# BaeHann/feature_level_style_transfer_for_TSC

Hardware: AMD Instinct MI355X
Metric: train-step samples/sec (univariate TS, len=512, batch=256) at 1/2/4/8 MI355X (higher is better)
Workload: dtype bf16x3

## Files before the change

### feature_level_style_transfer_for_tsc_amd/_lib.py

```python
from __future__ import annotations

import ctypes
import os
from ctypes import POINTER, Structure, c_char_p, c_float, c_int, c_int32, c_int64, c_void_p
from typing import Optional

import torch

ABI_VERSION = 21
_LIB_NAME = "libfst_hip.so"
_HERE = os.path.dirname(os.path.abspath(__file__))
LIB_PATH = os.environ.get("FST_HIP_LIB", os.path.join(_HERE, _LIB_NAME))


class FstLibraryError(RuntimeError):
    pass


class WSrc(Structure):
    _fields_ = [("w", c_void_p), ("off0", c_int64), ("sm", c_int64), ("sc", c_int64), ("st", c_int64)]


_P = c_void_p
_I32P = c_void_p
_SIGNATURES = {
    "fst_version": (c_int, []),
    "fst_last_error": (c_char_p, []),
    "fst_pack_weights": (c_int, [_I32P, _I32P, c_int, POINTER(WSrc), POINTER(WSrc), c_int, c_int, c_int, c_int, _P, c_void_p]),
    "fst_pack_weights_bf16x3": (c_int, [_I32P, _I32P, c_int, POINTER(WSrc), POINTER(WSrc), c_int, c_int, c_int, c_int, _P, c_void_p]),
    "fst_unpack_weights": (c_int, [_I32P, _I32P, c_int, _P, c_int, _P, c_int64, c_int64, c_int64, c_int64,
                                   _P, c_int64, c_int64, c_int64, c_int64, c_int, c_void_p]),
    "fst_mask_taps": (c_int, [_P, _I32P, _I32P, c_int, c_int, c_int, c_void_p]),
    "fst_conv_gemm": (c_int, [_P, c_int64, _P, c_int64, _P, _I32P, _I32P, c_int, _P, _P, c_int64, _P, c_int64,
                              _P, c_int64, c_int, c_int, c_int, c_int, c_int, c_int, c_int, c_int, c_void_p]),
    "fst_conv_wgrad": (c_int, [_P, c_int64, _P, c_int64, _P, c_int64, _P, c_int64, c_int, _P, _I32P, _I32P, c_int,
                               c_int, c_int, c_int, c_int, c_int, c_int64, c_void_p]),
    "fst_conv_last_route": (c_int, [POINTER(c_int32)]),
    "fst_row_sum": (c_int, [_P, c_int64, c_int, c_int, c_int, _P, c_void_p]),
    "fst_bn_stats": (c_int, [_P, c_int, c_int, c_int, _P, c_int64, c_void_p]),
    "fst_bn_finalize": (c_int, [_P, c_int, _P, _P, _P, _P, c_int, c_int, c_float, c_float, _P, c_void_p]),
    "fst_bn_apply": (c_int, [_P, _P, _P, _P, _P, c_int, c_int, c_int, c_int, c_int64, c_void_p]),
    "fst_bn_bwd_reduce": (c_int, [_P, _P, _P, _P, c_int, c_int, c_int, c_int, _P, c_int64, c_void_p]),
    "fst_bn_bwd_apply": (c_int, [_P, _P, _P, _P, _P, c_int, _P, _P, _P, c_int, c_int, c_int, c_int, c_int, c_int, c_int64, c_void_p]),
    "fst_bn_bwd_reduce_join": (c_int, [_P, _P, _P, _P, _P, c_int, c_int, c_int, _P, _P, c_int64, c_void_p]),
    "fst_bn_bwd_apply_join": (c_int, [_P, _P, _P, _P, _P, _P, _P, c_int, _P, _P, _P, _P, _P, _P, c_int, c_int, c_int, c_int, c_int,
                                      c_int64, c_void_p]),
    "fst_gate_fwd": (c_int, [_P, _P, c_int, c_int, c_int, c_int64, c_void_p]),
    "fst_gate_bwd": (c_int, [_P, _P, _P, c_int, c_int, c_int, c_int64, c_void_p]),
    "fst_coupling_sum_slots": (c_int64, [c_int, c_int, c_int]),
    "fst_coupling_fwd": (c_int, [_P, _P, _P, c_int, c_int, c_int, c_int64, _P, c_void_p]),
    "fst_coupling_bwd": (c_int, [_P, _P, _P, _P, _P, _P, _P, _P, c_int, c_int, c_int, c_int64, c_void_p]),
    "fst_coupling_inv_fwd": (c_int, [_P, _P, _P, c_int, c_int, c_int, c_int64, c_void_p]),
    "fst_coupling_inv_bwd": (c_int, [_P, _P, _P, _P, _P, c_int, c_int, c_int, c_int64, c_void_p]),
    "fst_rmsprop_multi": (c_int, [_P, _P, _P, _P, _P, c_int, c_float, c_float, c_void_p]),
    "fst_adam_multi": (c_int, [_P, _P, _P, _P, _P, c_int, _P, c_float, c_float, c_float, c_float, c_void_p]),
    "fst_rmsprop_multi_dev": (c_int, [_P, _P, _P, _P, _P, c_int, c_float, c_float, c_void_p]),
    "fst_adam_multi_dev": (c_int, [_P, _P, _P, _P, _P, c_int, _P, _P, c_float, c_float, c_float, c_void_p]),
# ... 129 lines not shown
```

### feature_level_style_transfer_for_tsc_amd/csrc/conv_engine.hip

```cpp
#include "fst_device.h"
#include <algorithm>
#include <type_traits>

struct ConvGemmParams {
  const float* x[2];
  long long x_bs[2];
  const float* a;
  const int32_t* plan;
  const float* bias;
  float* y;
  long long y_bs;
  const float* res;
  long long res_bs;
  float* y2;
  long long y2_bs;
  int msplit, m2_start;
  int B, L, M;
  int tiles_per_seq, ksplit, flags, mg_per_wg, ldw;
  int stage_vec;
  int epi_vec;
  int epi_lds_off;
};

template <int MB, int NB, int MODE>
// ... 439 lines not shown
    asm volatile("s_waitcnt vmcnt(0)" ::: "memory");
#endif
    FST_T(td);
    FST_ACC(3, tc, td);
    if (qn < ct.q_end) commit(buf ^ 1);
    FST_T(te);
    FST_ACC(4, td, te);
    __syncthreads();
    FST_T(tf);
    FST_ACC(5, te, tf);
    q = qn;
    buf ^= 1;
  }
  FST_T(tg);

  conv_epilogue<MB, NB>(p, acc, g, ct.b, ct.t0, ct.wave_n0, ct.half, ct.l31, p.bias != nullptr && blockIdx.z == 0, lds);
  FST_T(th);
  FST_ACC(6, tg, th);
  FST_ACC(7, ts0, th);
  FST_FLUSH(fst_stamps);
}

template <int MB, int NB>
__global__ __launch_bounds__(256, 2) void conv_gemm_bf3_kernel(ConvGemmParams p, const int32_t* __restrict__ plan) {
  extern __shared__ __attribute__((aligned(16))) float lds[];
  constexpr int TILE_N = 128 * NB;
  constexpr int NBLK = TILE_N / 32 + 1;
  constexpr int GS = NBLK * 1024 + 128;
  constexpr int A_BYTES = MB * 2048;
  constexpr int SLOT = A_BYTES + 2 * GS;
  constexpr int NA = A_BYTES / 1024;
  constexpr int NI = NA + 2 * NBLK;
  constexpr int NPW = (NI + 3) / 4;
  char* const ldsb = reinterpret_cast<char*>(lds);
  const PlanView pv = plan_view(plan);
  const ConvTile ct = conv_tile<TILE_N, NB>(p, pv);
  const int tid = ct.tid, lane = ct.lane, half = ct.half, l31 = ct.l31, b = ct.b, t0 = ct.t0, q_begin = ct.q_begin, q_end = ct.q_end,
            wave_n0 = ct.wave_n0;
  const int g = blockIdx.y;
  const int L = p.L;
  const int32_t* ent = pv.mg + 4 * (g * pv.n_chunks);
  const int wave_s = __builtin_amdgcn_readfirstlane(tid >> 6);
  const char* const zero16 = reinterpret_cast<const char*>(p.a) + (long long)pv.n_stages * A_BYTES;

  auto issue = [&](int q, int slot) {
    const int32_t* c = pv.chunk + 4 * q;
    const int32_t* e = ent + 4 * q;
    const int c_count = c[2];
    const char* asrc = reinterpret_cast<const char*>(p.a) + (long long)e[3] * A_BYTES;
    const float* xb = p.x[c[0]] + (long long)b * p.x_bs[c[0]] + (long long)c[1] * L;
    const int tbase = t0 - pv.pad_left + e[0] * pv.dil;
    const int t4 = tbase & ~3;
    const bool spill = (tbase & 3) != 0;
    char* const sl = ldsb + slot * SLOT;
#pragma unroll
    for (int i = 0; i < NPW; ++i) {
      const int idx = wave_s + 4 * i;
      if (idx >= NI) break;
      if (idx < NA) {
        lds_dma16(asrc + idx * 1024 + lane * 16, sl + idx * 1024);
      } else {
        const int bi = idx - NA;
        const int gq = bi >= NBLK ? 1 : 0, m = bi - gq * NBLK;
        const int row = 8 * gq + (lane >> 3);
        const int t = t4 + 32 * m + 4 * (lane & 7);
        bool ok = row < c_count && t >= 0 && t < L;
        if (m == NBLK - 1) ok = ok && spill && (lane & 7) == 0;
        const char* src = ok ? reinterpret_cast<const char*>(xb + ((long long)row * L + t)) : zero16;
        lds_dma16(src, sl + A_BYTES + gq * GS + m * 1024);
      }
    }
  };
  auto wait_stage = [&](int newer) {
    constexpr int R = NI % 4;
    const bool full = R == 0 || wave_s < R;
    if (newer == 0) wait_vmcnt<0>();
    else if (newer == 1) { if (full) wait_vmcnt<NPW>(); else wait_vmcnt<NPW - 1>(); }
    else { if (full) wait_vmcnt<2 * NPW>(); else wait_vmcnt<2 * NPW - 2>(); }
  };

  f32x16 acc[MB][NB];
  zero_acc(acc);

  FST_SUMS(8);
  FST_T(ts0);
  int q0 = next_live(ent, q_begin, q_end);
  int q1 = q0 < q_end ? next_live(ent, q0 + 1, q_end) : q_end;
  if (q0 < q_end) issue(q0, 0);
  if (q1 < q_end) issue(q1, 1);
  int slot = 0;
  FST_T(ts1);
  FST_ACC(0, ts0, ts1);
  while (q0 < q_end) {
    FST_T(ta);
    const int q2 = q1 < q_end ? next_live(ent, q1 + 1, q_end) : q_end;
    wait_stage(q1 < q_end ? 1 : 0);
    FST_T(tb);
    FST_ACC(1, ta, tb);
    __builtin_amdgcn_s_barrier();
    FST_T(tc);
    FST_ACC(2, tb, tc);
    if (q2 < q_end) issue(q2, slot >= 1 ? slot - 1 : 2);
    FST_T(td);
    FST_ACC(3, tc, td);
    const int sub = (t0 - pv.pad_left + ent[4 * q0] * pv.dil) & 3;
    const char* base = ldsb + slot * SLOT;
    bf16x8 bh[NB], bl[NB];
#pragma unroll
    for (int nb = 0; nb < NB; ++nb) {
      const int colx = wave_n0 + nb * 32 + l31 + sub;
      const char* bp = base + A_BYTES + half * GS + (colx >> 5) * 1024 + (colx & 31) * 4;
      float v[8];
#pragma unroll
      for (int j = 0; j < 8; ++j) v[j] = *reinterpret_cast<const float*>(bp + j * 128);
      split_bf16x8(v, bh[nb], bl[nb]);
    }
#ifdef FST_STAMPS
    asm volatile("" ::"v"(bh[0]), "v"(bl[0]), "v"(bh[NB - 1]), "v"(bl[NB - 1]));
#endif
    FST_T(te);
    FST_ACC(4, td, te);
#pragma unroll
    for (int mb = 0; mb < MB; ++mb) {
      bf16x8 ah, al;
      lds_read_a_frag(base, mb, lane, ah, al);
#pragma unroll
      for (int nb = 0; nb < NB; ++nb) mfma_bf3(acc[mb][nb], ah, al, bh[nb], bl[nb]);
    }
    FST_T(tf);
    FST_ACC(5, te, tf);
    q0 = q1;
    q1 = q2;
    slot = slot == 2 ? 0 : slot + 1;
  }
  FST_T(tg);
  __syncthreads();
  conv_epilogue<MB, NB>(p, acc, g, b, t0, wave_n0, half, l31, p.bias != nullptr && blockIdx.z == 0, lds);
  FST_T(th);
  FST_ACC(6, tg, th);
  FST_ACC(7, ts0, th);
  FST_FLUSH(fst_stamps);
}

template <int MB, int NB>
__global__ __launch_bounds__(256, 2) void conv_win_bf3_kernel(ConvGemmParams p, const int32_t* __restrict__ plan) {
  extern __shared__ __attribute__((aligned(16))) float lds[];
  constexpr int TILE_N = 128 * NB;
  char* const ldsb = reinterpret_cast<char*>(lds);
  const PlanView pv = plan_view(plan);
  const ConvTile ct = conv_tile<TILE_N, NB>(p, pv);
  const int g_begin = blockIdx.y * p.mg_per_wg;
  const int g_end = min(pv.n_mgroups, g_begin + p.mg_per_wg);
  const int slot_bytes = p.ldw * 64;

  const bool resident = p.stage_vec != 0;
  int jlo_all = 0, width_all = 0;
  if (resident) {
    conv_window_union(pv, ct.q_begin, ct.q_end, g_begin, g_end, TILE_N, jlo_all, width_all);
    for (int q = ct.q_begin; q < ct.q_end; ++q)
      stage_window_bf16(p, pv, ct, q, jlo_all, width_all, ldsb + (q - ct.q_begin) * slot_bytes);
    __syncthreads();
  }

// ... 376 lines not shown
                     fst_aligned16(res);
  ConvRoute r;
  if (int rc = conv_gemm_route(pv, ps, nb_cfg, L, ksplit, flags, in16, out16, res != nullptr, &r)) return rc;

  ConvGemmParams p;
  p.x[0] = x0; p.x[1] = x1; p.x_bs[0] = x0_bs; p.x_bs[1] = x1_bs;
  p.a = a_packed; p.plan = plan_dev; p.bias = bias;
  p.y = y; p.y_bs = y_bs; p.res = res; p.res_bs = res_bs; p.y2 = y2; p.y2_bs = y2_bs; p.msplit = msplit;
  p.m2_start = m2_start;
  p.B = B; p.L = L; p.M = M;
  p.tiles_per_seq = (L + 128 * nb_cfg - 1) / (128 * nb_cfg);
  p.ksplit = ksplit; p.flags = flags;
  p.mg_per_wg = r.mg_per_wg; p.ldw = r.ldw; p.stage_vec = r.stage_vec; p.epi_vec = r.epi_vec; p.epi_lds_off = r.epi_lds_off;
  if (r.lds_bytes > 48 * 1024)
    if (int rc = fst_allow_full_lds((const void*)r.fn, "fst_conv_gemm")) return rc;
  const bool rows = r.family == FST_ROUTE_WIN_ROWS;
  set_route(r.family, rows ? 0 : pv.MB, rows ? 0 : nb_cfg, r.vec, 0, 0, r.epi, ksplit);
  dim3 grid((unsigned)(B * p.tiles_per_seq), (unsigned)((pv.n_mgroups + r.mg_per_wg - 1) / r.mg_per_wg), (unsigned)ksplit);
  hipLaunchKernelGGL(r.fn, grid, dim3(256), r.lds_bytes, (hipStream_t)stream, p, plan_dev);
  FST_LAUNCH_CHECK();
  return 0;
}

struct WgradParams {
  const float* x[2];
  long long x_bs[2];
  const float* dy;
  long long dy_bs;
  const float* dy2;
  long long dy2_bs;
  int msplit;
  float* da;
  const int32_t* plan;
  int B, L, M, ksplit, tiles_per_seq, ldw, region_floats, n_regions;
  long long x0_mul_off;
  long long slab_floats;
};

#define WG_ITEMS 4

__device__ __forceinline__ int wg_wave_u(int tid) { return __builtin_amdgcn_readfirstlane(tid >> 6); }

template <int MBW, int TW, bool VEC, bool BF3>
struct WgDyStage {
  static constexpr int DYS = TW + 1;
  static constexpr int DYB = 2 * TW + 16;
// ... 682 lines not shown
```

### feature_level_style_transfer_for_tsc_amd/csrc/fst_device.h

```cpp
#pragma once
#include "fst_common.h"

typedef __bf16 bf16x8 __attribute__((ext_vector_type(8)));
typedef __bf16 bf16x2 __attribute__((ext_vector_type(2)));
typedef float f32x2 __attribute__((ext_vector_type(2)));
typedef unsigned u32x4 __attribute__((ext_vector_type(4)));
typedef float f32x16 __attribute__((ext_vector_type(16)));

__device__ __forceinline__ void split_bf16_pair(float a, float b, unsigned& hi, unsigned& lo) {
  const f32x2 v = {a, b};
  hi = __builtin_bit_cast(unsigned, __builtin_convertvector(v, bf16x2));
  const f32x2 r = {a - __uint_as_float(hi << 16), b - __uint_as_float(hi & 0xffff0000u)};
  lo = __builtin_bit_cast(unsigned, __builtin_convertvector(r, bf16x2));
}

__device__ __forceinline__ void split_bf16x8(const float (&v)[8], bf16x8& hi, bf16x8& lo) {
  u32x4 h, l;
#pragma unroll
  for (int j = 0; j < 4; ++j) {
    unsigned hh, ll;
    split_bf16_pair(v[2 * j], v[2 * j + 1], hh, ll);
    h[j] = hh; l[j] = ll;
  }
  hi = __builtin_bit_cast(bf16x8, h);
// ... 31 lines not shown
  asm volatile("s_waitcnt vmcnt(%0)" ::"n"(N) : "memory");
}

__device__ __forceinline__ void lds_dma16(const void* gsrc, void* lds_dst) {
  __builtin_amdgcn_global_load_lds((const __attribute__((address_space(1))) void*)gsrc, (__attribute__((address_space(3))) void*)lds_dst,
                                   16, 0, 0);
}

#ifdef FST_STAMPS
__device__ __forceinline__ unsigned long long fst_now() {
  unsigned long long t;
  asm volatile("s_memtime %0\n\ts_waitcnt lgkmcnt(0)" : "=s"(t)::"memory");
  return t;
}
template <int N>
int fst_read_stamps(unsigned long long (&counters)[N], unsigned long long* out_host, int reset) {
  if (out_host) hipMemcpyFromSymbol(out_host, HIP_SYMBOL(counters), sizeof(counters));
  if (reset) { unsigned long long z[N] = {0}; hipMemcpyToSymbol(HIP_SYMBOL(counters), z, sizeof(z)); }
  return 0;
}
#define FST_T(var) const unsigned long long var = fst_now()
#define FST_ACC(slot, a, b) fst_sum_[slot] += (b) - (a)
#define FST_SUMS(N) unsigned long long fst_sum_[N] = {0}
#define FST_FLUSH(counters) \
  if (lane == 0) for (int i_ = 0; i_ < (int)(sizeof(fst_sum_) / sizeof(fst_sum_[0])); ++i_) atomicAdd(&counters[i_], fst_sum_[i_])
#else
#define FST_T(var)
#define FST_ACC(slot, a, b)
#define FST_SUMS(N)
#define FST_FLUSH(counters)
#endif
```

### feature_level_style_transfer_for_tsc_amd/ops.py

```python
from __future__ import annotations

import ctypes
import math
import os
from typing import Callable, Dict, List, NamedTuple, Optional, Sequence, Tuple

import torch

from . import _lib
from . import dist as _dist
from ._lib import WSrc, check, ptr, stream_ptr
from .plan import Plan, Segment, build_plan, pick_mb

EPI_RELU, EPI_ACC2, EPI_ATOMIC, EPI_ACC1 = 1, 2, 4, 8
GEMM_BF16X3 = 16
WGRAD_SLABS = 32
MATH = os.environ.get("FST_MATH", "bf16x3")
LDS_BUDGET = 96 * 1024
LDS_MULTI_CHUNK = 44 * 1024
PIPE_C = 16

_PARTIAL_BACKWARD = False


# ... 206 lines not shown
        flags |= GEMM_BF16X3
    msplit = M if msplit is None else msplit
    m2_start = msplit if m2_start is None else m2_start
    x0_bs, _ = _ncl(x0, "x0")
    x1_bs = _ncl(x1, "x1")[0] if x1 is not None else 0
    y_bs = _ncl(y, "y")[0] if y is not None else 0
    res_bs = _ncl(res, "res")[0] if res is not None else 0
    y2_bs = _ncl(y2, "y2")[0] if y2 is not None else 0
    t0 = KERNEL_TIMER.begin() if KERNEL_TIMER is not None else None
    check(lib.fst_conv_gemm(ptr(x0), x0_bs, ptr(x1), x1_bs, ptr(a), ptr(plan.dev(x0.device)), plan.host_ptr(),
                            plan.length, ptr(bias), ptr(y), y_bs, ptr(res), res_bs, ptr(y2), y2_bs, msplit, m2_start, B, L,
                            M, nb, ksplit, flags, stream_ptr()), "fst_conv_gemm")
    if t0 is not None:
        key = route_kernel_name(last_route())
        if KERNEL_TIMER.detail:
            key += f" M={M} rec={plan.total_records} dil={plan.dil}"
        rows_in = x0.size(1) + (x1.size(1) if x1 is not None else 0) + (res.size(1) if res is not None else 0)
        rows_out = (msplit if y is not None else 0) + ((M - m2_start) if y2 is not None else 0)
        if y2 is not None and flags & EPI_ACC2:
            rows_in += M - m2_start
        if flags & EPI_ACC1 and y is not None:
            rows_in += msplit
        KERNEL_TIMER.end(key, t0, 2.0 * B * L * _plan_macs_per_step(plan, M), 4.0 * B * L * (rows_in + rows_out))


def conv_wgrad(plan: Plan, x0: Tensor, x1: Optional[Tensor], dy: Tensor, dy2: Optional[Tensor], msplit: int, B: int,
               L: int, M: int, ksplit: int, x0_mul_off: int = 0) -> Tensor:
    lib = _lib.load()
    n_slabs = max(1, min(ksplit, B * ((L + 31) // 32)))
    da = torch.empty(n_slabs, plan.packed_floats, device=x0.device, dtype=torch.float32)
    x0_bs, _ = _ncl(x0, "x0")
    x1_bs = _ncl(x1, "x1")[0] if x1 is not None else 0
    dy_bs, _ = _ncl(dy, "dy")
    dy2_bs = _ncl(dy2, "dy2")[0] if dy2 is not None else 0
    t0 = KERNEL_TIMER.begin() if KERNEL_TIMER is not None else None
    bf3 = MATH == "bf16x3"
    check(lib.fst_conv_wgrad(ptr(x0), x0_bs, ptr(x1), x1_bs, ptr(dy), dy_bs, ptr(dy2), dy2_bs, msplit, ptr(da),
                             ptr(plan.dev(x0.device)), plan.host_ptr(), plan.length, B, L, M, ksplit,
                             (GEMM_BF16X3 if bf3 else 0) | WGRAD_SLABS, x0_mul_off, stream_ptr()),
          "fst_conv_wgrad")
    if t0 is not None:
        key = route_kernel_name(last_route())
        if KERNEL_TIMER.detail:
            key += f" M={M} rec={plan.total_records} ksplit={ksplit}"
        rows_in = x0.size(1) + (x1.size(1) if x1 is not None else 0) + M
        KERNEL_TIMER.end(key, t0, 2.0 * B * L * _plan_macs_per_step(plan, M), 4.0 * B * L * rows_in + 8.0 * plan.packed_floats)
# ... 1220 lines not shown
                                        _ptr_table(da_out), rs_b, rs_d, ptr(do), h2, do.numel(), ptr(d_u0), d_u0_bs, nl, B, L, n, h,
                                        numel, stream_ptr()), "fst_wn_stack_bwd_proj")
    else:
        check(lib.fst_wn_stack_bwd(_ptr_table(ts_list), _ptr_table(imgs_b), _ptr_table(imgs_d), _ptr_table(dgs), _ptr_table(da_out),
                                   rs_b, rs_d, ptr(d_out), ptr(d_u0), d_u0_bs, nl, B, L, n, h, numel, stream_ptr()),
              "fst_wn_stack_bwd")
    if t0 is not None:
        sr = n if do is None else h2
        flops = 2.0 * B * L * (n * ((n + sr) * nl - n) + nl * 2 * n * (3 * n + h))
        rows = nl * (2 * n + sr + 2 * 2 * n + 2 * h) + n * sum(t is not None for t in da_out)
        KERNEL_TIMER.end("wn_stack_bwd_kernel", t0, flops, 4.0 * B * L * rows)


def _wn_layer(S: WNSpecs, ts: Sequence[Tensor], i: int):
    n, nl = S.n, S.n_layers
    rows = slice(2 * n * i, 2 * n * (i + 1))
    return ts[6 + i], ts[2][rows], ts[6 + nl + i], ts[3][rows], ts[6 + 2 * nl + i], ts[6 + 3 * nl + i]


def wn_infer_enabled() -> bool:
    return os.environ.get("FST_WN_INFER", "1") != "0"


def _wn_forward(specs: WNSpecs, u0: Tensor, flat: Tensor, save: bool = True):
    S, nl, n, h = specs, specs.n_layers, specs.n, specs.h
    flat = flat.contiguous()
    W = S.unflatten(flat)
    B, _, L = u0.shape
    dev = u0.device
    infer = not save and wn_infer_enabled()
    y0 = torch.empty(B, n, L, device=dev, dtype=torch.float32) if infer else empty_with_slack(B, n, L, dev)
    a = S.start.forward(u0, None, W[0], None, W[1], y=y0)
    fused = wn_fused_ok(n, h, L, a, u0, kernel=S.kernel)
    if fused:
        out = torch.empty(B, n, L, device=dev, dtype=torch.float32)
        imgs = wn_pack_layers([_wn_layer(S, W, i) for i in range(nl)], n, h)
        if infer:
            other = torch.empty_like(a) if nl > 1 else None
            a_list, ts_list = [a if i % 2 == 0 else other for i in range(nl)], None
        else:
            a_list = [a] + [empty_with_slack(B, n, L, dev) for _ in range(nl - 1)]
            ts_list = [torch.empty(B, 2 * n, L, device=dev, dtype=torch.float32) for _ in range(nl)]
        if wn_stack_fwd_ok(n, h, L, nl, B):
            _wn_stack_forward(not infer, a_list, u0, imgs, ts_list or (), out, n, h)
        else:
            for i in range(nl):
                last = i == nl - 1
                _wn_layer_forward(not infer, a_list[i], u0, imgs[i], ts_list[i] if ts_list else None, None,
                                  None if last else a_list[i + 1], out, i == 0, last, n, h, 2 ** i)
        if infer:
            return S.end.forward(out, None, W[4], None, W[5]), True, ()
        acts_list = ts_list
    else:
        lib = _lib.load()
        out = torch.zeros(B, n, L, device=dev, dtype=torch.float32)
        bias_g = torch.stack(W[6 + nl: 6 + 2 * nl]) + W[3].view(nl, 2 * n)
        a_list, ts_list, acts_list = [a], [], []
        for i in range(nl):
            in_w, cond_w, _, _, rs_w, rs_b = _wn_layer(S, W, i)
            g = S.ins[i].forward(a, u0, in_w, cond_w, bias_g[i])
            acts = torch.empty(B, n, L, device=dev, dtype=torch.float32)
            check(lib.fst_gate_fwd(ptr(g), ptr(acts), B, n, L, _gate_numel(acts, g), stream_ptr()), "fst_gate_fwd")
            ts_list.append(g)
            acts_list.append(acts)
            if i < nl - 1:
                a_next = torch.empty_like(a)
                S.rs[i].forward(acts, None, rs_w, None, rs_b, y=a_next, res=a, y2=out, msplit=n, flags=EPI_ACC2)
                a = a_next
                a_list.append(a)
            else:
                S.rs[i].forward(acts, None, rs_w, None, rs_b, y=None, y2=out, msplit=0, flags=EPI_ACC2)
    o = S.end.forward(out, None, W[4], None, W[5])
    return o, fused, (u0, out, *a_list, *ts_list, *acts_list, flat)


def _wn_backward(S: WNSpecs, fused: bool, sv, do: Tensor, d_u0: Tensor, need_w: bool, pool: Optional["WNGradPool"] = None):
    nl, h, n = S.n_layers, S.h, S.n
    u0, out, flat = sv[0], sv[1], sv[2 + 3 * nl]
    a_list, ts_list, acts_list = sv[2: 2 + nl], sv[2 + nl: 2 + 2 * nl], sv[2 + 2 * nl: 2 + 3 * nl]
    W = S.unflatten(flat)
    B, _, L = u0.shape
    deferring = need_w and pool is not None and fused and any(
        wn_wgrad_ok(0, B, L, n, h, 2 ** i, a_list[i]) or wn_wgrad_ok(1, B, L, n, h, 2 ** i) for i in range(nl))
    d_flat = (torch.zeros_like(flat) if deferring else torch.empty_like(flat)) if need_w else None
    G = S.unflatten(d_flat) if need_w else None
    do = do.contiguous()

    stack = fused and all(wn_dgrad_ok(n, h, 2 ** i) for i in range(nl)) and wn_stack_bwd_ok(n, h, L, nl)
    proj = stack and wn_skip_proj_ok(h, need_w)
    d_out = None if proj and not need_w else S.end.grad_x0(do, W[4])
    da_sums = None
    if need_w:
        S.end.grad_w(out, None, do, out0=G[4])
        row_sum(do, out=G[5])
        d_out_sum = row_sum(d_out, out=G[6 + 4 * nl - 1])
        o0 = S.offsets[6 + 3 * nl]
        d_rs_b = d_flat[o0: o0 + (nl - 1) * 2 * n].view(nl - 1, 2 * n)
        d_rs_b[:, n:] = d_out_sum
        da_sums = [G[1]] + [d_rs_b[i, :n] for i in range(nl - 1)]
    part_b = part_d = None
    if not fused:
        d_a = _wn_backward_unfused(S, W, G, a_list, ts_list, acts_list, u0, d_out, d_u0, da_sums)
    elif stack:
        d_a, part_b, part_d = _wn_backward_stack(S, W, G, a_list, ts_list, u0, d_out, d_u0, pool, do if proj else None)
    else:
        d_a, part_b, part_d = _wn_backward_layers(S, W, G, a_list, ts_list, u0, d_out, d_u0, da_sums, pool)
    S.start.grad_x0(d_a, W[0], out=d_u0, flags=EPI_ACC1)
    if need_w:
        S.start.grad_w(u0, None, d_a, out0=G[0])
        o0 = S.offsets[6 + nl]
        if part_b is not None:
            torch.sum(part_b[:, : 2 * n, :], dim=2, out=d_flat[o0: o0 + nl * 2 * n].view(nl, 2 * n))
        if part_d is not None:
            if nl > 1:
                torch.sum(part_d[1:, :n, :], dim=2, out=d_rs_b[:, :n])
            torch.sum(part_d[0, :n, :], dim=1, out=G[1])
        G[3].copy_(d_flat[o0: o0 + nl * 2 * n])
    return d_flat


def _wn_wgrad_rs(S: WNSpecs, i: int, d_a: Optional[Tensor], d_out: Tensor, ts: Tensor, G, pool) -> None:
    n, B, L, last, g_rs_w = S.n, d_out.size(0), d_out.size(2), i == S.n_layers - 1, _wn_layer(S, G, i)[4]
    if wn_wgrad_ok(1, B, L, n, S.h, 2 ** i):
        if pool is not None:
            pool.add((1, i), (d_a, d_out, ts))
        else:
            wn_wgrad_rs(d_a, d_out, ts, g_rs_w, last, n)
    elif last:
        S.rs[i].grad_w(ts[:, :n], None, d_out, x0_mul_off=n * L, out0=g_rs_w)
    else:
# ... 183 lines not shown

    @staticmethod
    def backward(ctx, dxn, d_o_ext, g_ls, g_sq):
        lib = _lib.load()
        keep, o = ctx.saved_tensors[0], ctx.saved_tensors[1]
        sv = ctx.saved_tensors[2:]
        S: WNSpecs = ctx.specs
        B, C, L = keep.shape
        if ctx.inverse:
            if dxn is None:
                dx, d_o = torch.zeros_like(keep), torch.zeros_like(o)
            else:
                dx, d_o = torch.empty_like(keep), torch.empty_like(o)
                dxn = dxn.contiguous()
                check(lib.fst_coupling_inv_bwd(ptr(keep), ptr(o), ptr(dxn), ptr(dx), ptr(d_o), B, S.h, L,
                                               _same_numel(keep, o, dxn, dx, d_o), stream_ptr()), "fst_coupling_inv_bwd")
        else:
            dx, d_o = _coupling_backward(keep, o, dxn, g_ls, g_sq)
        if d_o_ext is not None:
            d_o = d_o + d_o_ext
        need_w = ctx.needs_input_grad[2] and _want_weight_grad()
        d_flat = _wn_backward(S, ctx.fused, sv, d_o, dx[:, : S.h], need_w, ctx.pool)
        return None, (dx if ctx.needs_input_grad[1] else None), d_flat, None, None


class CouplingInvFn(torch.autograd.Function):

    @staticmethod
    def forward(ctx, x, o):
        lib = _lib.load()
        x, o = x.contiguous(), o.contiguous()
        B, C, L = x.shape
        xn = torch.empty_like(x)
        check(lib.fst_coupling_inv_fwd(ptr(x), ptr(o), ptr(xn), B, C // 2, L, _same_numel(x, o, xn), stream_ptr()),
              "fst_coupling_inv_fwd")
        ctx.save_for_backward(xn, o)
        return xn

    @staticmethod
    def backward(ctx, dxn):
        lib = _lib.load()
        xn, o = ctx.saved_tensors
        B, C, L = xn.shape
        dx, d_o = torch.empty_like(xn), torch.empty_like(o)
        dxn = dxn.contiguous()
        check(lib.fst_coupling_inv_bwd(ptr(xn), ptr(o), ptr(dxn), ptr(dx), ptr(d_o), B, C // 2, L,
# ... 322 lines not shown
```

### feature_level_style_transfer_for_tsc_amd/waveglow.py

```python
from __future__ import annotations

from typing import Dict, List, Tuple

import torch
import torch.nn as nn

from . import ops


class Invertible1x1Conv(nn.Module):

    def __init__(self, c: int):
        super().__init__()
        self.conv = nn.Conv1d(c, c, kernel_size=1, stride=1, padding=0, bias=False)
        W = torch.linalg.qr(torch.FloatTensor(c, c).normal_())[0]
        if torch.det(W) < 0:
            W[:, 0] = -1 * W[:, 0]
        self.conv.weight.data = W.contiguous().view(c, c, 1)
        self.spec = ops.ConvSpec(c, c)
        self._logdet_cache = None

    def forward(self, z: torch.Tensor, reverse: bool = False):
        batch_size, _, n_of_groups = z.size()
        if reverse:
            if not hasattr(self, "W_inverse"):
                self.W_inverse = self.conv.weight.detach().squeeze().float().inverse()[..., None].contiguous()
            return ops.conv1d(self.spec, z.contiguous(), self.W_inverse, None)
        W = self.conv.weight
        cache = self._logdet_cache
        if cache is not None and cache[0] is not None:
            logdet = cache[0]
            if len(cache) > 1 and cache[1] is not None:
                torch.cuda.current_stream().wait_event(cache[1])
                logdet.record_stream(torch.cuda.current_stream())
                cache[1] = None
        else:
            logdet = ops.logdet(W.squeeze())
            if cache is not None:
                cache[0] = logdet
        log_det_W = batch_size * n_of_groups * logdet
        return ops.conv1d(self.spec, z.contiguous(), W, None), log_det_W


def _wn_conv(cin: int, cout: int, k: int, **kw) -> nn.Conv1d:
    return nn.utils.weight_norm(nn.Conv1d(cin, cout, k, **kw), name="weight")


def _folded(conv: nn.Conv1d) -> torch.Tensor:
    return torch._weight_norm(conv.weight_v, conv.weight_g, 0)


class WN(nn.Module):

    def __init__(self, n_in_channels: int, n_layers: int, n_channels: int, kernel_size: int):
        super().__init__()
        self.n_layers, self.n_channels = n_layers, n_channels
        self.in_layers = nn.ModuleList()
        self.res_skip_layers = nn.ModuleList()
        self.start = _wn_conv(n_in_channels, n_channels, 1)
        end = nn.Conv1d(n_channels, 2 * n_in_channels, 1)
        end.weight.data.zero_()
        end.bias.data.zero_()
        self.end = end
        self.cond_layer = _wn_conv(n_in_channels, 2 * n_channels * n_layers, 1)
# ... 86 lines not shown
            for c in self.wg.convinv:
                c._logdet_cache = None
            return False

    def shared_fold(self):
        return WaveGlow._SharedFold(self)

    def prefetch_logdets(self, stream: "torch.cuda.Stream") -> None:
        if not self.convinv[0].conv.weight.is_cuda:
            return
        with torch.cuda.stream(stream):
            for c in self.convinv:
                if c._logdet_cache is not None and c._logdet_cache[0] is None:
                    c._logdet_cache[0] = ops.logdet(c.conv.weight.squeeze())
                    ev = torch.cuda.Event()
                    ev.record(stream)
                    c._logdet_cache.append(ev)

    def forward(self, forward_input: torch.Tensor):
        audio = forward_input
        log_s_list, log_det_W_list = [], []
        n_half = self.n_group // 2
        for k in range(self.n_flows):
            audio, log_det_W = self.convinv[k](audio)
            log_det_W_list.append(log_det_W)
            audio, output, s_ls, s_sq = ops.FlowFn.apply(self.WN[k].specs, audio, *self.WN[k]._folded_for(False))
            log_s = output[:, n_half:, :]
            log_s._fst_sum = s_ls
            audio._fst_sq_sum = s_sq
            log_s_list.append(log_s)
        return audio, log_s_list, log_det_W_list

    def infer(self, audio: torch.Tensor, sigma: float = 1.0) -> torch.Tensor:
        n_half = self.n_group // 2
        for k in reversed(range(self.n_flows)):
            audio = ops.FlowFn.apply(self.WN[k].specs, audio, *self.WN[k]._folded_for(True))[0]
            audio = self.convinv[k](audio, reverse=True)
        return audio


class WaveGlowLoss(nn.Module):

    def __init__(self, sigma: float = 1.0):
        super().__init__()
        self.sigma = sigma

    def forward(self, model_output):
        z, log_s_list, log_det_W_list = model_output
        total = lambda t, attr: getattr(t, attr) if hasattr(t, attr) else None
# ... 10 lines not shown
```

### include/fst_hip.h

```cpp
#ifndef FST_HIP_H
#define FST_HIP_H

#include <stdint.h>

#ifdef __cplusplus
extern "C" {
#endif

#define FST_ABI_VERSION 21

int fst_version(void);
const char* fst_last_error(void);

#define FST_PLAN_HEADER 16

typedef struct {
  const float* w;
  int64_t off0, sm, sc, st;
} fst_wsrc;

int fst_pack_weights(const int32_t* plan_dev, const int32_t* plan_host, int plan_len,
                     const fst_wsrc* src0_host, const fst_wsrc* src1_host,
                     int M, int g_begin, int g_end , int row_base ,
                     float* a_packed, void* stream);

int fst_pack_weights_bf16x3(const int32_t* plan_dev, const int32_t* plan_host, int plan_len,
                            const fst_wsrc* src0_host, const fst_wsrc* src1_host,
                            int M, int g_begin, int g_end, int row_base, void* a_image, void* stream);

int fst_unpack_weights(const int32_t* plan_dev, const int32_t* plan_host, int plan_len,
                       const float* a_packed, int M,
                       float* dw0, int64_t off0_0, int64_t sm0, int64_t sc0, int64_t st0,
                       float* dw1, int64_t off0_1, int64_t sm1, int64_t sc1, int64_t st1,
                       int n_slabs ,
                       void* stream);

int fst_mask_taps(float* w, const int32_t* live_lo, const int32_t* live_hi, int M, int C, int K, void* stream);

#define FST_EPI_RELU    1
#define FST_EPI_ACC2    2
#define FST_EPI_ATOMIC  4
#define FST_EPI_ACC1    8
#define FST_GEMM_BF16X3 16
#define FST_WGRAD_SLABS 32
int fst_conv_gemm(const float* x0, int64_t x0_bs, const float* x1, int64_t x1_bs,
                  const float* a_packed, const int32_t* plan_dev, const int32_t* plan_host, int plan_len,
                  const float* bias,
                  float* y, int64_t y_bs, const float* res, int64_t res_bs,
                  float* y2, int64_t y2_bs, int msplit, int m2_start ,
                  int B, int L, int M, int nb_cfg, int ksplit, int flags, void* stream);

int fst_conv_wgrad(const float* x0, int64_t x0_bs, const float* x1, int64_t x1_bs,
                   const float* dy, int64_t dy_bs, const float* dy2, int64_t dy2_bs, int msplit,
                   float* da_packed, const int32_t* plan_dev, const int32_t* plan_host, int plan_len,
                   int B, int L, int M, int ksplit, int flags , int64_t x0_mul_off, void* stream);

#define FST_ROUTE_GEMM      1
#define FST_ROUTE_PIPE      2
#define FST_ROUTE_BF3       3
#define FST_ROUTE_WIN_BF3   4
#define FST_ROUTE_WIN_ROWS  5
#define FST_ROUTE_WGRAD     6
#define FST_ROUTE_EPI_PLAIN   0
#define FST_ROUTE_EPI_ADD     1
#define FST_ROUTE_EPI_ATOMIC  2
#define FST_ROUTE_EPI_VEC     3
#define FST_ROUTE_EPI_VEC_ADD 4
int fst_conv_last_route(int32_t out[8]);

int fst_row_sum(const float* x, int64_t x_bs, int B, int C, int L, float* out, void* stream);

#define FST_BN_SLOTS 16
int fst_bn_stats(const float* y, int B, int C, int L, float* part , int64_t numel, void* stream);
// ... 210 lines not shown
```

Measured before the change: 3633.

## Fuse invertible 1x1 conv with WN start conv in one flow-chain kernel

Adds a flow_chain_bf3_kernel that runs the invertible 1x1 conv and the WaveNet start conv back to back in one kernel. The intermediate tile stays in LDS and feeds the second GEMM directly, and the conv output z is also written out. The backward pass uses the same kernel to chain the start-conv dgrad with the transposed invertible-conv dgrad, adding the passed-through dz rows. This removes a kernel launch and a global-memory round trip per flow step in both directions. The price is extra weight packing per call, a narrow shape gate, and extra LDS and register pressure.

Measured after the change: 3645, median of 4. About the same (+0.3%).

```diff
diff --git a/feature_level_style_transfer_for_tsc_amd/_lib.py b/feature_level_style_transfer_for_tsc_amd/_lib.py
--- a/feature_level_style_transfer_for_tsc_amd/_lib.py
+++ b/feature_level_style_transfer_for_tsc_amd/_lib.py
@@ -7,7 +7,7 @@
 
 import torch
 
-ABI_VERSION = 21
+ABI_VERSION = 22
 _LIB_NAME = "libfst_hip.so"
 _HERE = os.path.dirname(os.path.abspath(__file__))
 LIB_PATH = os.environ.get("FST_HIP_LIB", os.path.join(_HERE, _LIB_NAME))
@@ -33,6 +33,9 @@
     "fst_mask_taps": (c_int, [_P, _I32P, _I32P, c_int, c_int, c_int, c_void_p]),
     "fst_conv_gemm": (c_int, [_P, c_int64, _P, c_int64, _P, _I32P, _I32P, c_int, _P, _P, c_int64, _P, c_int64,
                               _P, c_int64, c_int, c_int, c_int, c_int, c_int, c_int, c_int, c_int, c_void_p]),
+    "fst_flow_chain_ok": (c_int, [c_int, c_int, c_int, c_int, c_int, c_int]),
+    "fst_flow_chain": (c_int, [_P, c_int64, _P, _I32P, _I32P, c_int, c_int, _P, c_int64, c_int, c_int, _P, c_int64, c_int,
+                               _P, _I32P, _I32P, c_int, _P, _P, c_int64, c_int, c_int, c_int, c_void_p]),
     "fst_conv_wgrad": (c_int, [_P, c_int64, _P, c_int64, _P, c_int64, _P, c_int64, c_int, _P, _I32P, _I32P, c_int,
                                c_int, c_int, c_int, c_int, c_int, c_int64, c_void_p]),
     "fst_conv_last_route": (c_int, [POINTER(c_int32)]),
diff --git a/feature_level_style_transfer_for_tsc_amd/csrc/conv_engine.hip b/feature_level_style_transfer_for_tsc_amd/csrc/conv_engine.hip
--- a/feature_level_style_transfer_for_tsc_amd/csrc/conv_engine.hip
+++ b/feature_level_style_transfer_for_tsc_amd/csrc/conv_engine.hip
@@ -485,8 +485,9 @@
 }
 
 template <int MB, int NB>
-__global__ __launch_bounds__(256, 2) void conv_gemm_bf3_kernel(ConvGemmParams p, const int32_t* __restrict__ plan) {
-  extern __shared__ __attribute__((aligned(16))) float lds[];
+__device__ __forceinline__ void conv_bf3_walk(const ConvGemmParams& p, const PlanView& pv, int g, int tid, int lane, int half,
+                                              int l31, int b, int t0, int q_begin, int q_end, int wave_n0, char* const ldsb,
+                                              f32x16 (&acc)[MB][NB] FST_SUMS_PARAM(8)) {
   constexpr int TILE_N = 128 * NB;
   constexpr int NBLK = TILE_N / 32 + 1;
   constexpr int GS = NBLK * 1024 + 128;
@@ -495,12 +496,6 @@
   constexpr int NA = A_BYTES / 1024;
   constexpr int NI = NA + 2 * NBLK;
   constexpr int NPW = (NI + 3) / 4;
-  char* const ldsb = reinterpret_cast<char*>(lds);
-  const PlanView pv = plan_view(plan);
-  const ConvTile ct = conv_tile<TILE_N, NB>(p, pv);
-  const int tid = ct.tid, lane = ct.lane, half = ct.half, l31 = ct.l31, b = ct.b, t0 = ct.t0, q_begin = ct.q_begin, q_end = ct.q_end,
-            wave_n0 = ct.wave_n0;
-  const int g = blockIdx.y;
   const int L = p.L;
   const int32_t* ent = pv.mg + 4 * (g * pv.n_chunks);
   const int wave_s = __builtin_amdgcn_readfirstlane(tid >> 6);
@@ -542,18 +537,14 @@
     else { if (full) wait_vmcnt<2 * NPW>(); else wait_vmcnt<2 * NPW - 2>(); }
   };
 
-  f32x16 acc[MB][NB];
-  zero_acc(acc);
-
-  FST_SUMS(8);
-  FST_T(ts0);
+  FST_T(tw0);
   int q0 = next_live(ent, q_begin, q_end);
   int q1 = q0 < q_end ? next_live(ent, q0 + 1, q_end) : q_end;
   if (q0 < q_end) issue(q0, 0);
   if (q1 < q_end) issue(q1, 1);
   int slot = 0;
   FST_T(ts1);
-  FST_ACC(0, ts0, ts1);
+  FST_ACC(0, tw0, ts1);
   while (q0 < q_end) {
     FST_T(ta);
     const int q2 = q1 < q_end ? next_live(ent, q1 + 1, q_end) : q_end;
@@ -596,12 +587,130 @@
     q1 = q2;
     slot = slot == 2 ? 0 : slot + 1;
   }
+}
+
+template <int MB, int NB>
+__global__ __launch_bounds__(256, 2) void conv_gemm_bf3_kernel(ConvGemmParams p, const int32_t* __restrict__ plan) {
+  extern __shared__ __attribute__((aligned(16))) float lds[];
+  const PlanView pv = plan_view(plan);
+  const ConvTile ct = conv_tile<128 * NB, NB>(p, pv);
+  const int tid = ct.tid, lane = ct.lane, half = ct.half, l31 = ct.l31, b = ct.b, t0 = ct.t0, q_begin = ct.q_begin, q_end = ct.q_end,
+            wave_n0 = ct.wave_n0;
+  const int g = blockIdx.y;
+  f32x16 acc[MB][NB];
+  zero_acc(acc);
+  FST_SUMS(8);
+  FST_T(ts0);
+  conv_bf3_walk<MB, NB>(p, pv, g, tid, lane, half, l31, b, t0, q_begin, q_end, wave_n0, reinterpret_cast<char*>(lds), acc FST_SUMS_ARG);
   FST_T(tg);
   __syncthreads();
   conv_epilogue<MB, NB>(p, acc, g, b, t0, wave_n0, half, l31, p.bias != nullptr && blockIdx.z == 0, lds);
   FST_T(th);
   FST_ACC(6, tg, th);
   FST_ACC(7, ts0, th);
+  FST_FLUSH(fst_stamps);
+}
+
+struct FlowChainParams {
+  ConvGemmParams g1, g2;
+  const float* e;
+  long long e_bs;
+  int e_rows, own;
+  float* y1;
+  long long y1_bs;
+  int y1_rows;
+};
+
+template <int MB1, int MB2, int NQ2, bool EXT>
+__global__ __launch_bounds__(256, 2) void flow_chain_bf3_kernel(FlowChainParams c, const int32_t* __restrict__ plan1,
+                                                                const int32_t* __restrict__ plan2) {
+  extern __shared__ __attribute__((aligned(16))) float lds[];
+  constexpr int NB = 2;
+  constexpr int ZG = 8 * 1024 + 128;
+  constexpr int ZROWS = 64;
+  static_assert(MB1 * 32 <= ZROWS && NQ2 * 16 <= ZROWS, "the assembled operand holds 64 rows");
+  char* const ldsb = reinterpret_cast<char*>(lds);
+  const PlanView pv1 = plan_view(plan1), pv2 = plan_view(plan2);
+  const ConvTile ct = conv_tile<128 * NB, NB>(c.g1, pv1);
+  const int tid = ct.tid, lane = ct.lane, half = ct.half, l31 = ct.l31, b = ct.b, t0 = ct.t0, wave_n0 = ct.wave_n0;
+  const int L = c.g1.L;
+  const int er = lane >> 4, ec = wave_n0 + (lane & 15) * 4;
+  const bool t_ok = t0 + ec < L;
+  float4 ev[EXT ? ZROWS / 4 : 1];
+  if constexpr (EXT) {
+    const float* eb = c.e + ((long long)b * c.e_bs + t0 + ec);
+#pragma unroll
+    for (int i = 0; i < ZROWS / 4; ++i) {
+      const int row = 4 * i + er;
+      ev[i] = (row < c.e_rows && t_ok) ? *reinterpret_cast<const float4*>(eb + (long long)row * L) : make_float4(0.f, 0.f, 0.f, 0.f);
+    }
+  }
+
+  f32x16 acc1[MB1][NB];
+  zero_acc(acc1);
+  FST_SUMS(8);
+  conv_bf3_walk<MB1, NB>(c.g1, pv1, 0, tid, lane, half, l31, b, t0, 0, pv1.n_chunks, wave_n0, ldsb, acc1 FST_SUMS_ARG);
+  __syncthreads();
+
+  bf16x8 a2h[NQ2][MB2], a2l[NQ2][MB2];
+#pragma unroll
+  for (int q = 0; q < NQ2; ++q) {
+    const char* src = reinterpret_cast<const char*>(c.g2.a) + (long long)pv2.mg[4 * q + 3] * (MB2 * 2048);
+#pragma unroll
+    for (int mb = 0; mb < MB2; ++mb) {
+      a2h[q][mb] = *reinterpret_cast<const bf16x8*>(src + mb * 2048 + lane * 16);
+      a2l[q][mb] = *reinterpret_cast<const bf16x8*>(src + mb * 2048 + 1024 + lane * 16);
+    }
+  }
+
+#pragma unroll
+  for (int mb = 0; mb < MB1; ++mb)
+#pragma unroll
+    for (int nb = 0; nb < NB; ++nb)
+#pragma unroll
+      for (int r = 0; r < 16; ++r) {
+        const int m = mb * 32 + (r & 3) + 8 * (r >> 2) + 4 * half, col = wave_n0 + nb * 32 + l31;
+        *reinterpret_cast<float*>(ldsb + (m >> 3) * ZG + (col >> 5) * 1024 + (m & 7) * 128 + (col & 31) * 4) = acc1[mb][nb][r] + 0.f;
+      }
+#pragma unroll
+  for (int i = 0; i < ZROWS / 4; ++i) {
+    const int row = 4 * i + er;
+    float* zp = reinterpret_cast<float*>(ldsb + (row >> 3) * ZG + (ec >> 5) * 1024 + (row & 7) * 128 + (ec & 31) * 4);
+    float4 v = *reinterpret_cast<const float4*>(zp);
+    float4 k = make_float4(0.f, 0.f, 0.f, 0.f);
+    if constexpr (EXT) {
+      if (row < c.own) {
+        v.x += 0.f + ev[i].x; v.y += 0.f + ev[i].y; v.z += 0.f + ev[i].z; v.w += 0.f + ev[i].w;
+      } else {
+        k = ev[i];
+      }
+    }
+    if (row < c.y1_rows && t_ok) *reinterpret_cast<float4*>(c.y1 + ((long long)b * c.y1_bs + (long long)row * L + t0 + ec)) = v;
+    if (row < c.own && t_ok) k = v;
+    *reinterpret_cast<float4*>(zp) = k;
+  }
+
+  f32x16 acc2[MB2][NB];
+  zero_acc(acc2);
+#pragma unroll
+  for (int q = 0; q < NQ2; ++q) {
+    bf16x8 bh[NB], bl[NB];
+#pragma unroll
+    for (int nb = 0; nb < NB; ++nb) {
+      const int colx = wave_n0 + nb * 32 + l31;
+      const char* bp = ldsb + (2 * q + half) * ZG + (colx >> 5) * 1024 + (colx & 31) * 4;
+      float v[8];
+#pragma unroll
+      for (int j = 0; j < 8; ++j) v[j] = *reinterpret_cast<const float*>(bp + j * 128);
+      split_bf16x8(v, bh[nb], bl[nb]);
+    }
+#pragma unroll
+    for (int mb = 0; mb < MB2; ++mb)
+#pragma unroll
+      for (int nb = 0; nb < NB; ++nb) mfma_bf3(acc2[mb][nb], a2h[q][mb], a2l[q][mb], bh[nb], bl[nb]);
+  }
+  __syncthreads();
+  conv_epilogue<MB2, NB>(c.g2, acc2, 0, b, t0, wave_n0, half, l31, c.g2.bias != nullptr, lds);
   FST_FLUSH(fst_stamps);
 }
 
@@ -1024,6 +1133,73 @@
   return 0;
 }
 
+static bool flow_chain_plan_ok(const PlanView& pv, const PlanScan& ps) {
+  if (!ps.pipeable || ps.needs_x1 || pv.n_mgroups != 1 || pv.ntaps != 1 || pv.pad_left != 0 || pv.chunk_cap != PIPE_C) return false;
+  for (int q = 0; q < pv.n_chunks; ++q) {
+    const int32_t *c = pv.chunk + 4 * q, *e = pv.mg + 4 * q;
+    if (c[0] != 0 || c[1] != PIPE_C * q || e[0] != 0 || e[1] != 1) return false;
+  }
+  return true;
+}
+
+typedef void (*flow_chain_fn)(FlowChainParams, const int32_t*, const int32_t*);
+
+extern "C" int fst_flow_chain_ok(int M1, int K1, int M2, int K2, int has_e, int L) {
+  if (L <= 0 || L % 4 != 0 || K1 <= 0) return 0;
+  if (!has_e) return M1 > 32 && M1 <= 64 && M2 > 64 && M2 <= 128 && K2 > 16 && K2 <= 32 && K2 <= M1;
+  return M1 > 0 && M1 <= 32 && M2 > 32 && M2 <= 64 && K2 > 48 && K2 <= 64 && K2 >= M1;
+}
+
+extern "C" int fst_flow_chain(const float* x, int64_t x_bs, const float* a1, const int32_t* plan1_dev, const int32_t* plan1_host,
+                              int plan1_len, int M1, const float* e, int64_t e_bs, int e_rows, int own, float* y1, int64_t y1_bs,
+                              int y1_rows, const float* a2, const int32_t* plan2_dev, const int32_t* plan2_host, int plan2_len,
+                              const float* bias2, float* y2, int64_t y2_bs, int M2, int B, int L, void* stream) {
+  if (int rc = fst_check_plan(plan1_host, plan1_len, M1, "fst_flow_chain")) return rc;
+  if (int rc = fst_check_plan(plan2_host, plan2_len, M2, "fst_flow_chain")) return rc;
+  const PlanView pv1 = plan_view(plan1_host), pv2 = plan_view(plan2_host);
+  const PlanScan ps1 = plan_scan(pv1), ps2 = plan_scan(pv2);
+  FST_REQUIRE(x && a1 && a2 && y2 && plan1_dev && plan2_dev, "fst_flow_chain: null operand");
+  FST_REQUIRE(B > 0 && L > 0 && L % 4 == 0, "fst_flow_chain: B=%d L=%d (L %% 4 == 0)", B, L);
+  FST_REQUIRE(flow_chain_plan_ok(pv1, ps1) && flow_chain_plan_ok(pv2, ps2),
+              "fst_flow_chain: both plans must be dense single-tap 16-channel stages of one input and one M-group");
+  const int K1 = ps1.rows_in[0], K2 = ps2.rows_in[0];
+  FST_REQUIRE(fst_flow_chain_ok(M1, K1, M2, K2, e != nullptr, L), "fst_flow_chain: no kernel for %d x %d then %d x %d%s", M1, K1,
+              M2, K2, e ? " with passed-through rows" : "");
+  FST_REQUIRE(own > 0 && own <= M1 && (e ? (e_rows == K2 && own <= e_rows) : own == K2),
+              "fst_flow_chain: own=%d e_rows=%d against M1=%d, K2=%d", own, e_rows, M1, K2);
+  FST_REQUIRE(y1_rows >= 0 && y1_rows <= M1 && (y1_rows == 0 || y1 != nullptr), "fst_flow_chain: y1_rows=%d, M1=%d", y1_rows, M1);
+  FST_REQUIRE(B == 1 || (x_bs >= (int64_t)K1 * L && y2_bs >= (int64_t)M2 * L && (!e || e_bs >= (int64_t)e_rows * L) &&
+                         (y1_rows == 0 || y1_bs >= (int64_t)y1_rows * L)),
+              "fst_flow_chain: a batch stride (x %lld, e %lld, y1 %lld, y2 %lld) is smaller than the rows it holds", (long long)x_bs,
+              (long long)e_bs, (long long)y1_bs, (long long)y2_bs);
+  FST_REQUIRE(x_bs % 4 == 0 && fst_aligned16(x) && (!e || (e_bs % 4 == 0 && fst_aligned16(e))) &&
+                  (y1_rows == 0 || (y1_bs % 4 == 0 && fst_aligned16(y1))),
+              "fst_flow_chain: x, e and y1 must be 16-byte aligned with batch strides of whole 16-byte pieces");
+
+  FlowChainParams c;
+  ConvGemmParams g = {};
+  g.L = L; g.B = B; g.ksplit = 1;
+  g.tiles_per_seq = (L + 255) / 256;
+  c.g1 = g;
+  c.g1.x[0] = x; c.g1.x_bs[0] = x_bs; c.g1.a = a1; c.g1.plan = plan1_dev; c.g1.M = M1;
+  c.g2 = g;
+  c.g2.a = a2; c.g2.plan = plan2_dev; c.g2.bias = bias2; c.g2.y = y2; c.g2.y_bs = y2_bs; c.g2.M = c.g2.msplit = c.g2.m2_start = M2;
+  c.g2.epi_vec = y2_bs % 4 == 0 && fst_aligned16(y2);
+  c.g2.epi_lds_off = 0;
+  c.e = e; c.e_bs = e_bs; c.e_rows = e ? e_rows : 0; c.own = own;
+  c.y1 = y1; c.y1_bs = y1_bs; c.y1_rows = y1_rows;
+  const flow_chain_fn fn = e ? flow_chain_bf3_kernel<1, 2, 4, true> : flow_chain_bf3_kernel<2, 4, 2, false>;
+  const int MB1 = e ? 1 : 2;
+  FST_REQUIRE(pv1.MB == MB1 && pv2.MB == (e ? 2 : 4) && pv2.n_chunks == (e ? 4 : 2),
+              "fst_flow_chain: plans of MB %d / %d and %d stages do not match the kernel instance", pv1.MB, pv2.MB, pv2.n_chunks);
+  const size_t ring = 3 * ((size_t)MB1 * 2048 + 2 * ((size_t)(256 / 32 + 1) * 1024 + 128));
+  const size_t lds_bytes = std::max(ring, (size_t)8 * (8 * 1024 + 128));
+  if (int rc = fst_allow_full_lds((const void*)fn, "fst_flow_chain")) return rc;
+  hipLaunchKernelGGL(fn, dim3((unsigned)(B * g.tiles_per_seq)), dim3(256), lds_bytes, (hipStream_t)stream, c, plan1_dev, plan2_dev);
+  FST_LAUNCH_CHECK();
+  return 0;
+}
+
 struct WgradParams {
   const float* x[2];
   long long x_bs[2];
diff --git a/feature_level_style_transfer_for_tsc_amd/csrc/fst_device.h b/feature_level_style_transfer_for_tsc_amd/csrc/fst_device.h
--- a/feature_level_style_transfer_for_tsc_amd/csrc/fst_device.h
+++ b/feature_level_style_transfer_for_tsc_amd/csrc/fst_device.h
@@ -77,11 +77,15 @@
 #define FST_T(var) const unsigned long long var = fst_now()
 #define FST_ACC(slot, a, b) fst_sum_[slot] += (b) - (a)
 #define FST_SUMS(N) unsigned long long fst_sum_[N] = {0}
+#define FST_SUMS_PARAM(N) , unsigned long long (&fst_sum_)[N]
+#define FST_SUMS_ARG , fst_sum_
 #define FST_FLUSH(counters) \
   if (lane == 0) for (int i_ = 0; i_ < (int)(sizeof(fst_sum_) / sizeof(fst_sum_[0])); ++i_) atomicAdd(&counters[i_], fst_sum_[i_])
 #else
 #define FST_T(var)
 #define FST_ACC(slot, a, b)
 #define FST_SUMS(N)
+#define FST_SUMS_PARAM(N)
+#define FST_SUMS_ARG
 #define FST_FLUSH(counters)
 #endif
diff --git a/feature_level_style_transfer_for_tsc_amd/ops.py b/feature_level_style_transfer_for_tsc_amd/ops.py
--- a/feature_level_style_transfer_for_tsc_amd/ops.py
+++ b/feature_level_style_transfer_for_tsc_amd/ops.py
@@ -252,6 +252,24 @@
         if flags & EPI_ACC1 and y is not None:
             rows_in += msplit
         KERNEL_TIMER.end(key, t0, 2.0 * B * L * _plan_macs_per_step(plan, M), 4.0 * B * L * (rows_in + rows_out))
+
+
+def flow_chain(plan1: Plan, a1: Tensor, x: Tensor, M1: int, own: int, plan2: Plan, a2: Tensor, bias2: Optional[Tensor], y2: Tensor,
+               M2: int, e: Optional[Tensor] = None, y1: Optional[Tensor] = None, y1_rows: int = 0) -> None:
+    lib = _lib.load()
+    B, L = x.size(0), x.size(2)
+    x_bs, _ = _ncl(x, "x")
+    e_bs = _ncl(e, "e")[0] if e is not None else 0
+    y1_bs = _ncl(y1, "y1")[0] if y1 is not None else 0
+    y2_bs, _ = _ncl(y2, "y2")
+    t0 = KERNEL_TIMER.begin() if KERNEL_TIMER is not None else None
+    check(lib.fst_flow_chain(ptr(x), x_bs, ptr(a1), ptr(plan1.dev(x.device)), plan1.host_ptr(), plan1.length, M1, ptr(e), e_bs,
+                             e.size(1) if e is not None else 0, own, ptr(y1), y1_bs, y1_rows, ptr(a2), ptr(plan2.dev(x.device)),
+                             plan2.host_ptr(), plan2.length, ptr(bias2), ptr(y2), y2_bs, M2, B, L, stream_ptr()), "fst_flow_chain")
+    if t0 is not None:
+        rows = x.size(1) + (e.size(1) if e is not None else 0) + y1_rows + M2
+        KERNEL_TIMER.end("flow_chain_bf3_kernel", t0, 2.0 * B * L * (_plan_macs_per_step(plan1, M1) + _plan_macs_per_step(plan2, M2)),
+                         4.0 * B * L * rows)
 
 
 def conv_wgrad(plan: Plan, x0: Tensor, x1: Optional[Tensor], dy: Tensor, dy2: Optional[Tensor], msplit: int, B: int,
@@ -1518,7 +1536,7 @@
     return os.environ.get("FST_WN_INFER", "1") != "0"
 
 
-def _wn_forward(specs: WNSpecs, u0: Tensor, flat: Tensor, save: bool = True):
+def _wn_forward(specs: WNSpecs, u0: Tensor, flat: Tensor, save: bool = True, start: Optional[Callable] = None):
     S, nl, n, h = specs, specs.n_layers, specs.n, specs.h
     flat = flat.contiguous()
     W = S.unflatten(flat)
@@ -1526,7 +1544,11 @@
     dev = u0.device
     infer = not save and wn_infer_enabled()
     y0 = torch.empty(B, n, L, device=dev, dtype=torch.float32) if infer else empty_with_slack(B, n, L, dev)
-    a = S.start.forward(u0, None, W[0], None, W[1], y=y0)
+    if start is not None:
+        start(y0, W[0], W[1])
+        a = y0
+    else:
+        a = S.start.forward(u0, None, W[0], None, W[1], y=y0)
     fused = wn_fused_ok(n, h, L, a, u0, kernel=S.kernel)
     if fused:
         out = torch.empty(B, n, L, device=dev, dtype=torch.float32)
@@ -1570,7 +1592,8 @@
     return o, fused, (u0, out, *a_list, *ts_list, *acts_list, flat)
 
 
-def _wn_backward(S: WNSpecs, fused: bool, sv, do: Tensor, d_u0: Tensor, need_w: bool, pool: Optional["WNGradPool"] = None):
+def _wn_backward(S: WNSpecs, fused: bool, sv, do: Tensor, d_u0: Tensor, need_w: bool, pool: Optional["WNGradPool"] = None,
+                 start_dgrad: Optional[Callable] = None):
     nl, h, n = S.n_layers, S.h, S.n
     u0, out, flat = sv[0], sv[1], sv[2 + 3 * nl]
     a_list, ts_list, acts_list = sv[2: 2 + nl], sv[2 + nl: 2 + 2 * nl], sv[2 + 2 * nl: 2 + 3 * nl]
@@ -1601,7 +1624,10 @@
         d_a, part_b, part_d = _wn_backward_stack(S, W, G, a_list, ts_list, u0, d_out, d_u0, pool, do if proj else None)
     else:
         d_a, part_b, part_d = _wn_backward_layers(S, W, G, a_list, ts_list, u0, d_out, d_u0, da_sums, pool)
-    S.start.grad_x0(d_a, W[0], out=d_u0, flags=EPI_ACC1)
+    if start_dgrad is not None:
+        start_dgrad(d_a, W[0])
+    else:
+        S.start.grad_x0(d_a, W[0], out=d_u0, flags=EPI_ACC1)
     if need_w:
         S.start.grad_w(u0, None, d_a, out0=G[0])
         o0 = S.offsets[6 + nl]
@@ -1831,6 +1857,77 @@
         need_w = ctx.needs_input_grad[2] and _want_weight_grad()
         d_flat = _wn_backward(S, ctx.fused, sv, d_o, dx[:, : S.h], need_w, ctx.pool)
         return None, (dx if ctx.needs_input_grad[1] else None), d_flat, None, None
+
+
+def flow_edges_ok(spec1: ConvSpec, S: WNSpecs, x: Tensor) -> bool:
+    if os.environ.get("FST_FLOW_EDGES", "1") == "0" or MATH != "bf16x3" or not x.is_cuda or x.dim() != 3:
+        return False
+    c, h, n, L = spec1.M, S.h, S.n, x.size(2)
+    if spec1.C0 != c or c != 2 * h or x.size(1) != c or x.dtype != torch.float32:
+        return False
+    lib = _lib.load()
+    return bool(lib.fst_flow_chain_ok(c, c, n, h, 0, L)) and bool(lib.fst_flow_chain_ok(h, n, c, c, 1, L))
+
+
+def _chain_image(spec: ConvSpec, plan: Plan, rows: int, w: Tensor, transposed: bool) -> Tensor:
+    if transposed:
+        return pack_weights(plan, rows, w, spec.s_w0_T(), bf3=True)
+    return pack_weights(plan, rows, w, spec.s_w0(), None, spec.s_w1(), bf3=True)
+
+
+class FlowStepFn(torch.autograd.Function):
+
+    @staticmethod
+    def forward(ctx, specs: WNSpecs, spec1: ConvSpec, x: Tensor, w1: Tensor, flat: Tensor, pool: Optional[WNGradPool] = None):
+        ctx.pool = pool
+        x = x.contiguous()
+        B, C, L = x.shape
+        h, n = specs.h, specs.n
+        z = torch.empty_like(x)
+
+        def start(y0: Tensor, w_start: Tensor, b_start: Tensor) -> None:
+            plan1 = spec1.fwd_plan(spec1.nb_for(B, L, spec1.mb, 0, 0))
+            plan2 = specs.start.fwd_plan(specs.start.nb_for(B, L, specs.start.mb, 0, 0))
+            flow_chain(plan1, _chain_image(spec1, plan1, C, w1, False), x, C, h, plan2,
+                       _chain_image(specs.start, plan2, n, w_start, False), b_start, y0, n, y1=z, y1_rows=C)
+
+        o, fused, saved = _wn_forward(specs, z[:, :h], flat, save=any(ctx.needs_input_grad), start=start)
+        xn, s_ls, s_sq = _coupling_forward(z, o)
+        ctx.specs, ctx.spec1, ctx.fused = specs, spec1, fused
+        if saved:
+            ctx.save_for_backward(x, w1, z, o, *saved)
+        ctx.set_materialize_grads(False)
+        return xn, o, s_ls, s_sq
+
+    @staticmethod
+    def backward(ctx, dxn, d_o_ext, g_ls, g_sq):
+        x, w1, z, o = ctx.saved_tensors[:4]
+        sv = ctx.saved_tensors[4:]
+        S: WNSpecs = ctx.specs
+        spec1: ConvSpec = ctx.spec1
+        B, C, L = z.shape
+        h, n = S.h, S.n
+        dz, d_o = _coupling_backward(z, o, dxn, g_ls, g_sq)
+        if d_o_ext is not None:
+            d_o = d_o + d_o_ext
+        need_w = ctx.needs_input_grad[4] and _want_weight_grad()
+        need_w1 = ctx.needs_input_grad[3] and _want_weight_grad(spec1)
+        dx = torch.empty_like(x) if ctx.needs_input_grad[2] else None
+
+        def start_dgrad(d_a: Tensor, w_start: Tensor) -> None:
+            plan1 = S.start.dx0_plan(S.start.nb_for(B, L, pick_mb(h), 0, 0))
+            plan2 = spec1.dx0_plan(spec1.nb_for(B, L, pick_mb(C), 0, 0))
+            flow_chain(plan1, _chain_image(S.start, plan1, h, w_start, True), d_a, h, h, plan2,
+                       _chain_image(spec1, plan2, C, w1, True), None, dx, C, e=dz, y1=dz if need_w1 else None,
+                       y1_rows=h if need_w1 else 0)
+
+        d_flat = _wn_backward(S, ctx.fused, sv, d_o, dz[:, :h], need_w, ctx.pool, start_dgrad if dx is not None else None)
+        dw1 = spec1.grad_w(x, None, dz)[0] if need_w1 else None
+        return None, None, dx, dw1, d_flat, None
+
+
+def flow_step(specs: WNSpecs, spec1: ConvSpec, x: Tensor, w1: Tensor, flat: Tensor, pool: Optional[WNGradPool] = None):
+    return FlowStepFn.apply(specs, spec1, x, w1 if torch.is_grad_enabled() else w1.detach(), flat, pool)
 
 
 class CouplingInvFn(torch.autograd.Function):
diff --git a/feature_level_style_transfer_for_tsc_amd/waveglow.py b/feature_level_style_transfer_for_tsc_amd/waveglow.py
--- a/feature_level_style_transfer_for_tsc_amd/waveglow.py
+++ b/feature_level_style_transfer_for_tsc_amd/waveglow.py
@@ -26,6 +26,10 @@
             if not hasattr(self, "W_inverse"):
                 self.W_inverse = self.conv.weight.detach().squeeze().float().inverse()[..., None].contiguous()
             return ops.conv1d(self.spec, z.contiguous(), self.W_inverse, None)
+        log_det_W = self.log_det(batch_size, n_of_groups)
+        return ops.conv1d(self.spec, z.contiguous(), self.conv.weight, None), log_det_W
+
+    def log_det(self, batch_size: int, n_of_groups: int) -> torch.Tensor:
         W = self.conv.weight
         cache = self._logdet_cache
         if cache is not None and cache[0] is not None:
@@ -38,8 +42,7 @@
             logdet = ops.logdet(W.squeeze())
             if cache is not None:
                 cache[0] = logdet
-        log_det_W = batch_size * n_of_groups * logdet
-        return ops.conv1d(self.spec, z.contiguous(), W, None), log_det_W
+        return batch_size * n_of_groups * logdet
 
 
 def _wn_conv(cin: int, cout: int, k: int, **kw) -> nn.Conv1d:
@@ -172,9 +175,15 @@
         log_s_list, log_det_W_list = [], []
         n_half = self.n_group // 2
         for k in range(self.n_flows):
-            audio, log_det_W = self.convinv[k](audio)
-            log_det_W_list.append(log_det_W)
-            audio, output, s_ls, s_sq = ops.FlowFn.apply(self.WN[k].specs, audio, *self.WN[k]._folded_for(False))
+            conv = self.convinv[k]
+            if ops.flow_edges_ok(conv.spec, self.WN[k].specs, audio):
+                log_det_W_list.append(conv.log_det(audio.size(0), audio.size(2)))
+                flat, _, pool = self.WN[k]._folded_for(False)
+                audio, output, s_ls, s_sq = ops.flow_step(self.WN[k].specs, conv.spec, audio, conv.conv.weight, flat, pool)
+            else:
+                audio, log_det_W = conv(audio)
+                log_det_W_list.append(log_det_W)
+                audio, output, s_ls, s_sq = ops.FlowFn.apply(self.WN[k].specs, audio, *self.WN[k]._folded_for(False))
             log_s = output[:, n_half:, :]
             log_s._fst_sum = s_ls
             audio._fst_sq_sum = s_sq
diff --git a/include/fst_hip.h b/include/fst_hip.h
--- a/include/fst_hip.h
+++ b/include/fst_hip.h
@@ -7,7 +7,7 @@
 extern "C" {
 #endif
 
-#define FST_ABI_VERSION 21
+#define FST_ABI_VERSION 22
 
 int fst_version(void);
 const char* fst_last_error(void);
@@ -49,6 +49,12 @@
                   float* y, int64_t y_bs, const float* res, int64_t res_bs,
                   float* y2, int64_t y2_bs, int msplit, int m2_start ,
                   int B, int L, int M, int nb_cfg, int ksplit, int flags, void* stream);
+
+int fst_flow_chain_ok(int M1, int K1, int M2, int K2, int has_e, int L);
+int fst_flow_chain(const float* x, int64_t x_bs, const float* a1, const int32_t* plan1_dev, const int32_t* plan1_host, int plan1_len,
+                   int M1, const float* e, int64_t e_bs, int e_rows, int own, float* y1, int64_t y1_bs, int y1_rows,
+                   const float* a2, const int32_t* plan2_dev, const int32_t* plan2_host, int plan2_len, const float* bias2,
+                   float* y2, int64_t y2_bs, int M2, int B, int L, void* stream);
 
 int fst_conv_wgrad(const float* x0, int64_t x0_bs, const float* x1, int64_t x1_bs,
                    const float* dy, int64_t dy_bs, const float* dy2, int64_t dy2_bs, int msplit,
```
